# sevagh/xumx-sliCQ

Hardware: NVIDIA B200
Metric: sliCQT fwd+inv audio-sec/sec (higher is better)
Workload: dtype f32

## Files before the change

xumx_slicq_b200/csrc/slicq_api.cu:

```cuda
#include "slicq_common.cuh"
#include "../../include/slicq.h"

#include <math.h>
#include <stdio.h>
#include <stdlib.h>
#include <string.h>
#include <string>
#include <vector>
#include <algorithm>
#include <atomic>
#include <mutex>

#ifdef SLICQ_EMU
#include <condition_variable>
#include <mutex>
#include <thread>
thread_local dim3 threadIdx;
dim3 blockIdx, blockDim, gridDim;
static unsigned char slicq_emu_smem_buf[256 * 1024] __attribute__((aligned(16)));
unsigned char* slicq_emu_smem = slicq_emu_smem_buf;
namespace {
struct EmuBarrier {
    std::mutex m; std::condition_variable cv; int count = 0, gen = 0, n = 1;
    void wait() {
// ... 42 lines not shown
std::mutex g_prof_mutex;
#endif
struct ProfScope {
#ifndef SLICQ_EMU
    int kid; cudaStream_t s; cudaEvent_t a, b; bool on;
    ProfScope(int k, cudaStream_t st) : kid(k), s(st), on(g_prof) {
        if (on) { cudaEventCreate(&a); cudaEventCreate(&b); cudaEventRecord(a, s); }
    }
    ~ProfScope() {
        if (on) { cudaEventRecord(b, s); ProfRec r; r.kid = kid; r.a = a; r.b = b; std::lock_guard<std::mutex> lk(g_prof_mutex); g_prof_recs.push_back(r); }
    }
#else
    ProfScope(int, cudaStream_t) {}
#endif
};

int fail(int code, const std::string& msg) {
    g_err = msg;
    return code;
}

struct FftPlan { int M, kind, A, B, cost; };
const FftPlan kFftPlans[] = {
#define SLICQ_FFT_SIZE(M_, K_, A_, B_, C_) {M_, K_, A_, B_, C_},
#include "fft_sizes.inc"
#undef SLICQ_FFT_SIZE
};

const FftPlan* find_fft_plan(int M) {
    for (size_t i = 0; i < sizeof(kFftPlans) / sizeof(kFftPlans[0]); ++i)
        if (kFftPlans[i].M == M) return &kFftPlans[i];
    return nullptr;
}

int fft_smem_per_transform(const FftPlan& f) {
    if (f.kind == 1) return (f.M + 1) * 8;
    if (f.kind == 2) {
        const int bp = (f.B % 2 == 0) ? f.B + 1 : f.B;
        const int ap = (f.A % 2 == 0) ? f.A + 1 : f.A;
        const int a = f.A * bp, b = f.B * ap;
        return (a > b ? a : b) * 8;
    }
    return (f.M + f.A) * 8;
}

int fft_threads_per_transform(const FftPlan& f) {
    if (f.kind == 1) return 1;
    if (f.kind == 2) return f.B;
    return f.B * (f.A <= 41 ? 2 : (f.A <= 61 ? 3 : 4));
}

struct Bucket {
    int M, first_bin, n_bins, gt, tw_off, kind, A, B, smem_per_fft;
    int gap_first, gap_n;
    double cost;
};

template <class T> int upload(const std::vector<T>& h, const T** d, std::vector<void*>& owned) {
    void* p = nullptr;
    if (cudaMalloc(&p, h.size() * sizeof(T)) != cudaSuccess) return -1;
    if (cudaMemcpy(p, h.data(), h.size() * sizeof(T), cudaMemcpyHostToDevice) != cudaSuccess) return -1;
    owned.push_back(p);
    *d = reinterpret_cast<const T*>(p);
    return 0;
}

}

#define SLICQ_MAX_WAYS 8
struct slicq_plan {
    int L, N2, hop, J, sum_M;
    std::vector<int> bin_M, bin_pos, bin_coff;
    std::vector<Bucket> buckets;
    SlicqDeviceTables dev;
    std::vector<void*> owned;
    int bins_smem;
    int pad_l, pad_r;
    long long spec_stride_fwd;
    long long t_stride;
    long long chunk_bytes;
    int target_jobs;
    int min_iters;
    int only_bucket;
    long long split_units;
    int split_ways;
    mutable cudaStream_t side[SLICQ_MAX_WAYS];
    mutable cudaEvent_t ev_fork, ev_join[SLICQ_MAX_WAYS];
    mutable bool side_ready;
    mutable std::mutex split_mutex;
};

extern "C" int slicq_abi_version(void) { return SLICQ_ABI_VERSION; }
#ifdef SLICQ_EMU
extern "C" int slicq_build_kind(void) { return 1; }
#else
extern "C" int slicq_build_kind(void) { return 0; }
#endif
extern "C" const char* slicq_last_error(void) { return g_err.c_str(); }
extern "C" int64_t slicq_launch_count(void) { return g_launches.load(); }

extern "C" int slicq_profile_enable(int on) { g_prof = on != 0; return SLICQ_OK; }

extern "C" int slicq_profile_read(double* ms, int64_t* launches) {
    for (int i = 0; i < K_COUNT; ++i) { if (ms) ms[i] = 0.0; if (launches) launches[i] = 0; }
#ifndef SLICQ_EMU
    std::lock_guard<std::mutex> lk(g_prof_mutex);
    for (ProfRec& r : g_prof_recs) {
        float t = 0.f;
        if (cudaEventSynchronize(r.b) == cudaSuccess && cudaEventElapsedTime(&t, r.a, r.b) == cudaSuccess) {
            if (ms) ms[r.kid] += t;
            if (launches) launches[r.kid] += 1;
        }
        cudaEventDestroy(r.a); cudaEventDestroy(r.b);
    }
    g_prof_recs.clear();
#endif
    return SLICQ_OK;
}

extern "C" void slicq_plan_destroy(slicq_plan* p) {
    if (!p) return;
    if (p->side_ready) {
        for (int h = 0; h < SLICQ_MAX_WAYS; ++h) { cudaStreamDestroy(p->side[h]); cudaEventDestroy(p->ev_join[h]); }
        cudaEventDestroy(p->ev_fork);
    }
    for (void* q : p->owned) cudaFree(q);
    delete p;
}

extern "C" int slicq_plan_create(const slicq_tables* t, slicq_plan** out) {
    if (!t || !out) return fail(SLICQ_E_INVALID, "null argument");
    *out = nullptr;
    const int L = t->sl_len, J = t->n_bins;
    if (L <= 0 || L % 4 != 0) return fail(SLICQ_E_INVALID, "sl_len must be a positive multiple of 4");
    if (J < 2 || !t->bin_M || !t->bin_pos || !t->win_fwd || !t->win_inv || !t->tukey)
        return fail(SLICQ_E_INVALID, "missing tables");
    if (slicq_slice_smem_bytes(L) < 0) {
        char buf[160];
        snprintf(buf, sizeof buf, "slice length %d does not fit the slice kernels' shared memory (two buffers of sl_len/2 complex numbers)", L);
        return fail(SLICQ_E_UNSUPPORTED, buf);
    }
    slicq_plan* p = new slicq_plan();
    p->L = L; p->N2 = L / 2; p->hop = L / 2; p->J = J;
    p->bin_M.assign(t->bin_M, t->bin_M + J);
    p->bin_pos.assign(t->bin_pos, t->bin_pos + J);
    p->bin_coff.resize(J);
    int off = 0;
    for (int j = 0; j < J; ++j) {
        const int M = p->bin_M[j], pos = p->bin_pos[j];
        if (M < 4 || M % 4 != 0 || M > SLICQ_MAX_M || !find_fft_plan(M)) {
            delete p;
            return fail(SLICQ_E_UNSUPPORTED, "bin length M must be a multiple of 4 in [16, 292]");
        }
        if (pos % 2 != 0 || pos < 0 || pos > p->N2 || (j > 0 && pos <= p->bin_pos[j - 1])) {
            delete p;
            return fail(SLICQ_E_UNSUPPORTED, "bin positions must be even, increasing and within [0, L/2]");
        }
        p->bin_coff[j] = off;
        off += M;
    }
    p->sum_M = off;
    for (int j = 1; j < J - 1; ++j) {
        if (p->bin_pos[j] + p->bin_M[j] / 2 > p->N2) {
            delete p;
            return fail(SLICQ_E_UNSUPPORTED, "a bin below Nyquist reaches beyond it: the mirrored-bin pass above Nyquist is not implemented");
        }
    }
    int tw_off = 0;
    for (int j = 0; j < J; ++j) {
        if (!p->buckets.empty() && p->buckets.back().M == p->bin_M[j]) {
            p->buckets.back().n_bins++;
            continue;
        }
        const FftPlan* f = find_fft_plan(p->bin_M[j]);
        Bucket b;
        b.M = p->bin_M[j]; b.first_bin = j; b.n_bins = 1; b.tw_off = tw_off;
        b.kind = f->kind; b.A = f->A; b.B = f->B; b.smem_per_fft = fft_smem_per_transform(*f);
        b.gt = 1; b.cost = 0.0; b.gap_first = 0; b.gap_n = 0;
        tw_off += b.M;
        p->buckets.push_back(b);
    }
    if ((int)p->buckets.size() > SLICQ_MAX_BUCKETS) {
        delete p;
        return fail(SLICQ_E_UNSUPPORTED, "too many buckets");
    }
    p->bins_smem = 0;
    for (Bucket& b : p->buckets) {
        const FftPlan* f = find_fft_plan(b.M);
        const int nthr = slicq_bins_threads();
        int gt = nthr / (b.n_bins * fft_threads_per_transform(*f));
        if (gt < 1) gt = 1;
        static const int stage_kb = getenv("SLICQ_BINS_STAGE_KB") ? atoi(getenv("SLICQ_BINS_STAGE_KB")) : 48;
        while (gt > 1 && b.n_bins * gt * b.smem_per_fft > stage_kb * 1024) --gt;
        if (b.n_bins * fft_threads_per_transform(*f) > nthr) {
            delete p;
            return fail(SLICQ_E_UNSUPPORTED, "bucket has too many bins for one CTA");
        }
        b.gt = gt;
        const int sm = b.n_bins * gt * b.smem_per_fft + 4096 + (f->kind == 1 ? b.n_bins * b.M * 4 + b.n_bins * 12 + 32 : 0) + (f->kind == 3 ? b.n_bins * 12 + 16 : 0) +
                       (f->kind >= 2 ? b.M * 8 + b.n_bins * b.M * 4 + b.n_bins * 4 + 16 : 0);
        if (sm > p->bins_smem) p->bins_smem = sm;
        b.cost = (double)b.n_bins * f->cost;
    }

    std::vector<float> wf(p->sum_M), wi(p->sum_M), tuk(t->tukey, t->tukey + L);
    int pad_l = 0, pad_r = 0;
    for (int j = 0; j < J; ++j) {
        const int M = p->bin_M[j], o = p->bin_coff[j];
        const double sgn = ((p->bin_pos[j] / 2) % 2) ? -1.0 : 1.0;
        for (int mc = 0; mc < M; ++mc) {
            const int m = (mc + M / 2) % M;
            wf[o + mc] = (float)((double)t->win_fwd[o + m] * sgn / (double)M);
            wi[o + mc] = (float)((double)t->win_inv[o + m] * sgn * (double)M / (double)L);
        }
        pad_l = std::max(pad_l, M / 2 - p->bin_pos[j]);
        pad_r = std::max(pad_r, p->bin_pos[j] + M / 2 - 1 - p->N2);
    }
    pad_l = (pad_l + 1) & ~1;
    pad_r = (pad_r + 1) & ~1;
    if (pad_l > p->N2 / 2 || pad_r > p->N2 / 2) {
        delete p;
        return fail(SLICQ_E_UNSUPPORTED, "bins reach too far beyond DC / Nyquist");
    }
    p->pad_l = pad_l; p->pad_r = pad_r;
    int tw_lo = 0, tw_hi = L;
    while (tw_lo < L && tuk[tw_lo] == 0.f) ++tw_lo;
    while (tw_hi > tw_lo && tuk[tw_hi - 1] == 0.f) --tw_hi;
    std::vector<float2> post(p->N2 / 2 + 1), tw(tw_off);
    for (int k = 0; k <= p->N2 / 2; ++k) {
        const double a = -2.0 * M_PI * (double)k / (double)L;
        post[k] = make_float2((float)cos(a), (float)sin(a));
    }
    for (const Bucket& b : p->buckets)
        for (int j = 0; j < b.M; ++j) {
            const double a = -2.0 * M_PI * (double)j / (double)b.M;
            tw[b.tw_off + j] = make_float2((float)cos(a), (float)sin(a));
        }
    const int N2 = p->N2;
    const int pl_off = pad_l;
    const int pl_len = (pl_off + N2 + 2 + std::max(pad_r, 2) + 1) & ~1;
    std::vector<int> toff(J), ov(J, 0), ovoff(J, 0);
    int n_ovf = 0;
    for (int j = 0; j < J; ++j) {
        const int lo = p->bin_pos[j] - p->bin_M[j] / 2;
        toff[j] = (j & 1) * pl_len + pl_off + lo;
        if (j >= 2) {
            const int end_prev = p->bin_pos[j - 2] + p->bin_M[j - 2] / 2;
            ov[j] = std::max(0, end_prev - lo);
        }
        if (ov[j] > p->bin_M[j] || (ov[j] & 1)) { delete p; return fail(SLICQ_E_UNSUPPORTED, "unsupported overlap between bins of one plane"); }
        if (j >= 4 && p->bin_pos[j - 4] + p->bin_M[j - 4] / 2 > lo) { delete p; return fail(SLICQ_E_UNSUPPORTED, "more than 4 bins overlap at one spectrum position"); }
        ovoff[j] = 2 * pl_len + n_ovf;
        n_ovf += ov[j];
    }
    for (const Bucket& b : p->buckets)
        for (int j = b.first_bin; j < b.first_bin + b.n_bins; ++j)
            if ((b.kind == 2 && ov[j] > b.A) || (b.kind == 3 && ov[j] > b.B)) { delete p; return fail(SLICQ_E_UNSUPPORTED, "overlap between bins of one plane exceeds the first transform pass"); }
    p->t_stride = (2LL * pl_len + n_ovf + 1) & ~1LL;
    std::vector<int4> ex;
    {
        const bool fold = (t->flags & SLICQ_PLAN_ADJOINT_OF_ANALYSIS) != 0;
        std::vector<int> e0(N2 + 1, -1), e1(N2 + 1, -1), c0(N2 + 1, -1), c1(N2 + 1, -1);
        for (int j = 0; j < J; ++j)
            for (int m = 0; m < ov[j]; ++m) {
                int f = p->bin_pos[j] - p->bin_M[j] / 2 + m;
                const bool out = f < 0 || f > N2;
                if (out && !fold) continue;
                if (f < 0) f = -f;
                if (f > N2) f = 2 * N2 - f;
                std::vector<int>& a = out ? c0 : e0;
                std::vector<int>& b = out ? c1 : e1;
                if (a[f] < 0) a[f] = ovoff[j] + m;
                else if (b[f] < 0) b[f] = ovoff[j] + m;
                else { delete p; return fail(SLICQ_E_UNSUPPORTED, "more than two overflow entries at one spectrum position"); }
            }
        for (int f = 0; f <= N2; ++f)
            if (e0[f] >= 0) ex.push_back(int4{f, e0[f], e1[f], 0});
        for (int f = 0; f <= N2; ++f)
            if (c0[f] >= 0) ex.push_back(int4{f, c0[f], c1[f], 1});
        if (L == kTunedSliceLen && ex.size() > 0 && ex.back().w) {
            delete p;
            return fail(SLICQ_E_UNSUPPORTED, "adjoint of the analysis: overflow below DC / above Nyquist is not implemented in "
                                             "the tuned slice kernels (slice length 18060)");
        }
    }
    const int n_ex = (int)ex.size();
    if (ex.empty()) ex.push_back(int4{0, 0, -1, 0});
    std::vector<int2> gaps;
    {
        std::vector<std::vector<int2> > per_bucket(p->buckets.size());
        auto bucket_of = [&](int j) { for (size_t i = 0; i < p->buckets.size(); ++i) if (j >= p->buckets[i].first_bin && j < p->buckets[i].first_bin + p->buckets[i].n_bins) return (int)i; return 0; };
        for (int q = 0; q < 2; ++q) {
            std::vector<int> owner(pl_len, -1);
            int last = -1;
            for (int j = q; j < J; j += 2) {
                const int lo = std::max(0, pl_off + p->bin_pos[j] - p->bin_M[j] / 2), hi = std::min(pl_len, pl_off + p->bin_pos[j] + p->bin_M[j] / 2);
                for (int f = lo; f < hi; ++f) owner[f] = j;
                last = j;
            }
            if (last < 0) { delete p; return fail(SLICQ_E_UNSUPPORTED, "a bin plane is empty"); }
            for (int f = 0; f < pl_len;) {
                if (owner[f] >= 0) { ++f; continue; }
                int g = f;
                while (g < pl_len && owner[g] < 0) ++g;
                const int next = g < pl_len ? owner[g] : last;
                per_bucket[bucket_of(next)].push_back(int2{q * pl_len + f, g - f});
                f = g;
            }
        }
        for (size_t i = 0; i < p->buckets.size(); ++i) {
            p->buckets[i].gap_first = (int)gaps.size();
// ... 113 lines not shown
    const int64_t hh = p->L / 4;
    const int64_t nblk = (T + hh - 1) / hh;
    return (nblk + 1) / 2 + 1;
}

namespace {
long long bytes_per_unit(const slicq_plan* p, int inverse) {
    if (!inverse) return p->spec_stride_fwd * 8;
    return p->t_stride * 8;
}
long long chunk_units(const slicq_plan* p, int inverse) {
    long long c = p->chunk_bytes / bytes_per_unit(p, inverse);
    if (c >= 296) c -= c % 296;
    return c < 1 ? 1 : c;
}
}

namespace {
bool use_split(const slicq_plan* p, int64_t n_rows, int64_t n_slices) {
    return p->split_units > 0 && n_rows >= 2 && n_rows * n_slices >= p->split_units;
}
int split_ways(const slicq_plan* p, int64_t n_rows) { return (int)(n_rows < p->split_ways ? n_rows : p->split_ways); }
int64_t part_row0(int64_t n_rows, int ways, int h) { return n_rows * h / ways; }
size_t half_scratch(const slicq_plan* p, int64_t rows, int64_t n_slices, int inverse) {
    long long units = rows * n_slices;
    const long long c = chunk_units(p, inverse);
    if (units > c) units = c;
    return ((size_t)(units * bytes_per_unit(p, inverse)) + 511) & ~(size_t)255;
}
int ensure_side_streams(const slicq_plan* p) {
    if (p->side_ready) return 0;
    if (cudaEventCreateWithFlags(&p->ev_fork, cudaEventDisableTiming)) return -1;
    for (int h = 0; h < SLICQ_MAX_WAYS; ++h)
        if (cudaStreamCreateWithFlags(&p->side[h], cudaStreamNonBlocking) || cudaEventCreateWithFlags(&p->ev_join[h], cudaEventDisableTiming))
            return -1;
    p->side_ready = true;
    return 0;
}
}

extern "C" size_t slicq_scratch_bytes(const slicq_plan* p, int64_t n_rows, int64_t n_slices, int inverse) {
    if (!p || n_rows <= 0 || n_slices <= 0) return 0;
    if (use_split(p, n_rows, n_slices)) {
        const int ways = split_ways(p, n_rows);
        size_t total = 256;
        for (int h = 0; h < ways; ++h)
            total += half_scratch(p, part_row0(n_rows, ways, h + 1) - part_row0(n_rows, ways, h), n_slices, inverse);
        return total;
    }
    return half_scratch(p, n_rows, n_slices, inverse) + 256;
}

namespace {
int fill_bins_params(const slicq_plan* p, const slicq_bucket_view* views, SlicqBinsParams& bp, int n_rs,
                     const slicq_bucket_view* masks = nullptr, const slicq_bucket_view* norms = nullptr) {
    int jobs = 0;
    bp.n_buckets = (int)p->buckets.size();
    double total = 0.0;
    for (const Bucket& b : p->buckets) total += b.cost;
    const int target = p->target_jobs > 0 ? p->target_jobs : std::min(4440, std::max(1184, 4 * n_rs));
    for (size_t i = 0; i < p->buckets.size(); ++i) {
        const Bucket& b = p->buckets[i];
        SlicqBucketArg& a = bp.b[i];
        a.ptr = reinterpret_cast<float2*>(views[i].ptr);
        a.s_row = views[i].s_row; a.s_bin = views[i].s_bin; a.s_slice = views[i].s_slice;
        a.M = b.M; a.first_bin = b.first_bin; a.n_bins = b.n_bins; a.gt = b.gt; a.tw_off = b.tw_off;
        a.gap_first = b.gap_first; a.gap_n = b.gap_n;
        a.mptr = masks ? reinterpret_cast<const float*>(masks[i].ptr) : nullptr;
        a.nptr = norms ? reinterpret_cast<float*>(norms[i].ptr) : nullptr;
        const slicq_bucket_view* aux = masks ? masks : norms;
        a.ms_row = aux ? aux[i].s_row : 0; a.ms_bin = aux ? aux[i].s_bin : 0; a.ms_slice = aux ? aux[i].s_slice : 0;
        if (p->only_bucket >= 0 && (int)i != p->only_bucket) {
            a.units_per_job = b.gt; a.n_jobs = 0; a.job_start = jobs;
            continue;
        }
        const int groups = (n_rs + b.gt - 1) / b.gt;
        int nj = (int)(target * b.cost / total + 0.5);
        if (nj > groups / p->min_iters) nj = groups / p->min_iters;
        if (nj < 1) nj = 1;
        const int gpj = (groups + nj - 1) / nj;
        a.units_per_job = gpj * b.gt;
        a.n_jobs = (n_rs + a.units_per_job - 1) / a.units_per_job;
        a.job_start = jobs;
        jobs += a.n_jobs;
    }
    return jobs;
}
}

namespace {
int forward_one(const slicq_plan* p, const float* x, int64_t n_rows, int64_t x_row_stride,
                int64_t n_samples, int64_t t0, int64_t k0, int64_t n_slices,
                const slicq_bucket_view* buckets, const slicq_bucket_view* norms, void* scratch, cudaStream_t s);
int inverse_one(const slicq_plan* p, const slicq_bucket_view* buckets, const slicq_bucket_view* masks, int64_t x_rows,
                int64_t n_rows, int64_t n_slices, int64_t k0, float* y, int64_t y_row_stride, int64_t length,
                int64_t t0, float* halo_out, void* scratch, cudaStream_t s);

template <class F>
int run_split(const slicq_plan* p, int64_t n_rows, int64_t n_slices, int inverse, void* scratch, cudaStream_t s, F fn) {
    std::lock_guard<std::mutex> lock(p->split_mutex);
    if (ensure_side_streams(p)) return fail(SLICQ_E_CUDA, "cannot create internal streams");
    const int ways = split_ways(p, n_rows);
    unsigned char* base = reinterpret_cast<unsigned char*>(scratch);
    cudaEventRecord(p->ev_fork, s);
    int rc = 0;
    for (int h = 0; h < ways && rc == 0; ++h) {
        const int64_t r0 = part_row0(n_rows, ways, h), rows = part_row0(n_rows, ways, h + 1) - r0;
        cudaStreamWaitEvent(p->side[h], p->ev_fork, 0);
        rc = fn(r0, rows, base, p->side[h]);
        base += half_scratch(p, rows, n_slices, inverse);
        cudaEventRecord(p->ev_join[h], p->side[h]);
        cudaStreamWaitEvent(s, p->ev_join[h], 0);
    }
    return rc;
}
}

namespace {
int forward_impl(const slicq_plan* p, const float* x, int64_t n_rows, int64_t x_row_stride,
                 int64_t n_samples, int64_t t0, int64_t k0, int64_t n_slices,
                 const slicq_bucket_view* buckets, const slicq_bucket_view* norms, void* scratch, size_t scratch_bytes,
                 void* stream) {
    if (!p || !x || !buckets) return fail(SLICQ_E_INVALID, "null argument");
    if (n_rows <= 0 || n_slices <= 0 || n_samples < 0) return fail(SLICQ_E_INVALID, "bad shape");
    if (n_rows * n_slices > 0x7fffffffLL) return fail(SLICQ_E_INVALID, "too many (row,slice) units");
    if (scratch_bytes < slicq_scratch_bytes(p, n_rows, n_slices, 0) || !scratch)
        return fail(SLICQ_E_SCRATCH, "scratch buffer too small (see slicq_scratch_bytes)");
    if (reinterpret_cast<uintptr_t>(scratch) & 15) return fail(SLICQ_E_SCRATCH, "scratch buffer must be 16-byte aligned");
    for (size_t i = 0; i < p->buckets.size(); ++i)
        if (!buckets[i].ptr || (norms && !norms[i].ptr)) return fail(SLICQ_E_INVALID, "null bucket pointer");
    cudaStream_t s0 = reinterpret_cast<cudaStream_t>(stream);
    if (use_split(p, n_rows, n_slices)) {
        return run_split(p, n_rows, n_slices, 0, scratch, s0, [&](int64_t r0, int64_t rows, void* scr, cudaStream_t st) {
            std::vector<slicq_bucket_view> v(buckets, buckets + p->buckets.size()), nv;
            for (auto& b : v) b.ptr = reinterpret_cast<float2*>(b.ptr) + r0 * b.s_row;
            if (norms) {
                nv.assign(norms, norms + p->buckets.size());
                for (auto& b : nv) b.ptr = reinterpret_cast<float*>(b.ptr) + r0 * b.s_row;
            }
            return forward_one(p, x + r0 * x_row_stride, rows, x_row_stride, n_samples, t0, k0, n_slices, v.data(),
                               norms ? nv.data() : nullptr, scr, st);
        });
    }
    return forward_one(p, x, n_rows, x_row_stride, n_samples, t0, k0, n_slices, buckets, norms, scratch, s0);
}
}

extern "C" int slicq_forward(const slicq_plan* p, const float* x, int64_t n_rows, int64_t x_row_stride,
                             int64_t n_samples, int64_t t0, int64_t k0, int64_t n_slices,
                             const slicq_bucket_view* buckets, void* scratch, size_t scratch_bytes, void* stream) {
    return forward_impl(p, x, n_rows, x_row_stride, n_samples, t0, k0, n_slices, buckets, nullptr, scratch, scratch_bytes, stream);
}

extern "C" int slicq_forward_norm(const slicq_plan* p, const float* x, int64_t n_rows, int64_t x_row_stride,
                                  int64_t n_samples, int64_t t0, int64_t k0, int64_t n_slices,
                                  const slicq_bucket_view* buckets, const slicq_bucket_view* norms, void* scratch,
                                  size_t scratch_bytes, void* stream) {
    if (!norms) return fail(SLICQ_E_INVALID, "norms missing");
    return forward_impl(p, x, n_rows, x_row_stride, n_samples, t0, k0, n_slices, buckets, norms, scratch, scratch_bytes, stream);
}

namespace {
int forward_one(const slicq_plan* p, const float* x, int64_t n_rows, int64_t x_row_stride,
                int64_t n_samples, int64_t t0, int64_t k0, int64_t n_slices,
                const slicq_bucket_view* buckets, const slicq_bucket_view* norms, void* scratch, cudaStream_t s) {
    const long long units = n_rows * n_slices, cu = chunk_units(p, 0);
    float2* H = reinterpret_cast<float2*>((reinterpret_cast<uintptr_t>(scratch) + 255) & ~(uintptr_t)255);
    SlicqSliceParams sp;
    memset(&sp, 0, sizeof sp);
    sp.t = p->dev; sp.x = const_cast<float*>(x); sp.x_row_stride = x_row_stride; sp.T = n_samples; sp.t0 = t0; sp.k0 = k0;
    sp.spec = H; sp.spec_stride = p->spec_stride_fwd; sp.S = (int)n_slices;
    SlicqBinsParams* bp = new SlicqBinsParams();
    bp->t = p->dev; bp->spec = H; bp->spec_stride = p->spec_stride_fwd; bp->S = (int)n_slices;
    bp->k0 = (int)k0;
    int rc = 0;
    for (long long u0 = 0; u0 < units && rc == 0; u0 += cu) {
        const int n = (int)((units - u0 < cu) ? (units - u0) : cu);
        sp.n_rs = n; sp.rs0 = (int)u0;
        { ProfScope ps(K_SLICE_FWD, s); rc = slicq_launch_slice_fwd(&sp, s); }
        ++g_launches;
        if (rc) break;
        bp->n_rs = n; bp->rs0 = (int)u0;
        const int jobs = fill_bins_params(p, buckets, *bp, n, nullptr, norms);
        { ProfScope ps(K_BINS_FWD, s); rc = slicq_launch_bins(bp, jobs, p->bins_smem, 0, s); }
        ++g_launches;
        if (rc) break;
        if ((p->dev.adjoint & 1) && p->dev.n_mir > 0) {
            rc = slicq_launch_mirror_adj(bp, s);
            ++g_launches;
        }
    }
    delete bp;
    if (rc) {
        char buf[128];
        snprintf(buf, sizeof buf, "kernel launch failed: %s", rc > 0 ? cudaGetErrorString((cudaError_t)rc) : "unsupported");
        return fail(SLICQ_E_CUDA, buf);
    }
    return SLICQ_OK;
}
}

namespace {
std::vector<slicq_bucket_view> packed_views(const slicq_plan* p, void* base_, int64_t n_rows, int64_t n_slices, size_t elem) {
    std::vector<slicq_bucket_view> v(p->buckets.size());
    unsigned char* base = reinterpret_cast<unsigned char*>(base_);
    for (size_t i = 0; i < p->buckets.size(); ++i) {
        const Bucket& b = p->buckets[i];
        v[i].ptr = base;
        v[i].s_slice = b.M;
        v[i].s_bin = (int64_t)n_slices * b.M;
        v[i].s_row = (int64_t)b.n_bins * n_slices * b.M;
        base += (size_t)n_rows * b.n_bins * n_slices * b.M * elem;
    }
    return v;
}
}

extern "C" int slicq_forward_packed(const slicq_plan* p, const float* x, int64_t n_rows, int64_t x_row_stride,
                                    int64_t n_samples, int64_t t0, int64_t k0, int64_t n_slices, void* coefs,
                                    void* scratch, size_t scratch_bytes, void* stream) {
    if (!p || !coefs) return fail(SLICQ_E_INVALID, "null argument");
    std::vector<slicq_bucket_view> v = packed_views(p, coefs, n_rows, n_slices, 8);
    return slicq_forward(p, x, n_rows, x_row_stride, n_samples, t0, k0, n_slices, v.data(), scratch, scratch_bytes, stream);
}

extern "C" int slicq_forward_packed_norm(const slicq_plan* p, const float* x, int64_t n_rows, int64_t x_row_stride,
                                         int64_t n_samples, int64_t t0, int64_t k0, int64_t n_slices, void* coefs,
                                         void* norms, void* scratch, size_t scratch_bytes, void* stream) {
    if (!p || !coefs || !norms) return fail(SLICQ_E_INVALID, "null argument");
    std::vector<slicq_bucket_view> v = packed_views(p, coefs, n_rows, n_slices, 8);
    std::vector<slicq_bucket_view> nv = packed_views(p, norms, n_rows, n_slices, 4);
    return slicq_forward_norm(p, x, n_rows, x_row_stride, n_samples, t0, k0, n_slices, v.data(), nv.data(), scratch,
                              scratch_bytes, stream);
}

namespace {
// ... 1 lines not shown
                 int64_t n_rows, int64_t n_slices, int64_t k0, float* y, int64_t y_row_stride, int64_t length,
                 int64_t t0, float* halo_out, void* scratch, size_t scratch_bytes, void* stream) {
    if (!p || (!y && length > 0) || !buckets) return fail(SLICQ_E_INVALID, "null argument");
    if (n_rows <= 0 || n_slices <= 0 || length < 0) return fail(SLICQ_E_INVALID, "bad shape");
    if (n_rows * n_slices > 0x7fffffffLL) return fail(SLICQ_E_INVALID, "too many (row,slice) units");
    if (scratch_bytes < slicq_scratch_bytes(p, n_rows, n_slices, 1) || !scratch)
        return fail(SLICQ_E_SCRATCH, "scratch buffer too small (see slicq_scratch_bytes)");
    if (reinterpret_cast<uintptr_t>(scratch) & 15) return fail(SLICQ_E_SCRATCH, "scratch buffer must be 16-byte aligned");
    for (size_t i = 0; i < p->buckets.size(); ++i)
        if (!buckets[i].ptr) return fail(SLICQ_E_INVALID, "null bucket pointer");
    cudaStream_t s0 = reinterpret_cast<cudaStream_t>(stream);
    bool split = use_split(p, n_rows, n_slices);
    if (split && masks) {
        const int ways = split_ways(p, n_rows);
        for (int h = 1; h < ways; ++h) split = split && (part_row0(n_rows, ways, h) % x_rows == 0);
    }
    if (split) {
        return run_split(p, n_rows, n_slices, 1, scratch, s0, [&](int64_t r0, int64_t rows, void* scr, cudaStream_t st) {
            std::vector<slicq_bucket_view> v(buckets, buckets + p->buckets.size()), mv;
            if (masks) {
                mv.assign(masks, masks + p->buckets.size());
                for (auto& b : mv) b.ptr = reinterpret_cast<float*>(b.ptr) + r0 * b.s_row;
            } else {
                for (auto& b : v) b.ptr = reinterpret_cast<float2*>(b.ptr) + r0 * b.s_row;
            }
            return inverse_one(p, v.data(), masks ? mv.data() : nullptr, x_rows, rows, n_slices, k0, y + r0 * y_row_stride,
                               y_row_stride, length, t0, halo_out ? halo_out + r0 * p->hop : nullptr, scr, st);
        });
    }
    return inverse_one(p, buckets, masks, x_rows, n_rows, n_slices, k0, y, y_row_stride, length, t0, halo_out, scratch, s0);
}

int inverse_one(const slicq_plan* p, const slicq_bucket_view* buckets, const slicq_bucket_view* masks, int64_t x_rows,
                int64_t n_rows, int64_t n_slices, int64_t k0, float* y, int64_t y_row_stride, int64_t length,
                int64_t t0, float* halo_out, void* scratch, cudaStream_t s) {
    const long long units = n_rows * n_slices, cu = chunk_units(p, 1);
    const long long nu = units < cu ? units : cu;
    unsigned char* base = reinterpret_cast<unsigned char*>((reinterpret_cast<uintptr_t>(scratch) + 255) & ~(uintptr_t)255);
    float2* T = reinterpret_cast<float2*>(base);
    (void)nu;
    SlicqBinsParams* bp = new SlicqBinsParams();
    bp->t = p->dev; bp->spec = T; bp->spec_stride = p->t_stride; bp->S = (int)n_slices;
    bp->x_rows = masks ? (int)x_rows : 0;
    bp->k0 = (int)k0;
    SlicqSliceParams sp;
    memset(&sp, 0, sizeof sp);
    sp.t = p->dev; sp.k0 = k0; sp.spec = T; sp.spec_stride = p->t_stride; sp.S = (int)n_slices;
    sp.x = y; sp.x_row_stride = y_row_stride; sp.T = length; sp.t0 = t0; sp.halo_out = halo_out;
    int rc = 0;
    for (long long u0 = 0; u0 < units && rc == 0;) {
        long long n = (units - u0 < cu) ? (units - u0) : cu;
        while (n > 1 && u0 + n < units && ((u0 + n) % n_slices) != 0 && (((u0 + n) % n_slices) & 1) == 0) --n;
        bp->n_rs = (int)n; bp->rs0 = (int)u0;
        const int jobs = fill_bins_params(p, buckets, *bp, (int)n, masks);
        { ProfScope ps(K_BINS_INV, s); rc = slicq_launch_bins(bp, jobs, p->bins_smem, 1, s); }
        ++g_launches;
        if (rc) break;
        if (p->dev.n_mir > 0) {
            rc = slicq_launch_mirror_fix(bp, s);
            ++g_launches;
            if (rc) break;
        }
        sp.n_rs = (int)n; sp.rs0 = (int)u0;
        {
            ProfScope ps(K_SLICE_INV, s);
            sp.parity = 0; rc = slicq_launch_slice_inv(&sp, s);
            if (!rc) { sp.parity = 1; rc = slicq_launch_slice_inv(&sp, s); }
        }
        g_launches += 2;
        u0 += n;
    }
    delete bp;
    if (rc) {
        char buf[128];
        snprintf(buf, sizeof buf, "kernel launch failed: %s", rc > 0 ? cudaGetErrorString((cudaError_t)rc) : "unsupported");
        return fail(SLICQ_E_CUDA, buf);
    }
    return SLICQ_OK;
}
}

extern "C" int slicq_inverse(const slicq_plan* p, const slicq_bucket_view* buckets, int64_t n_rows,
                             int64_t n_slices, int64_t k0, float* y, int64_t y_row_stride, int64_t length,
                             int64_t t0, float* halo_out, void* scratch, size_t scratch_bytes, void* stream) {
    return inverse_impl(p, buckets, nullptr, 0, n_rows, n_slices, k0, y, y_row_stride, length, t0, halo_out,
                        scratch, scratch_bytes, stream);
}

extern "C" int slicq_inverse_masked(const slicq_plan* p, const slicq_bucket_view* mix, const slicq_bucket_view* masks,
                                    int64_t n_targets, int64_t n_rows, int64_t n_slices, int64_t k0, float* y,
                                    int64_t y_row_stride, int64_t length, int64_t t0, float* halo_out, void* scratch,
                                    size_t scratch_bytes, void* stream) {
    if (!masks || n_targets <= 0) return fail(SLICQ_E_INVALID, "masks / n_targets missing");
    if (p) for (size_t i = 0; i < p->buckets.size(); ++i)
        if (!masks[i].ptr) return fail(SLICQ_E_INVALID, "null mask pointer");
    return inverse_impl(p, mix, masks, n_rows, n_targets * n_rows, n_slices, k0, y, y_row_stride, length, t0, halo_out,
                        scratch, scratch_bytes, stream);
}
```

xumx_slicq_b200/csrc/slicq_fft_tile.cuh:

```cuda
#pragma once
#include "slicq_common.cuh"
#include "dft_codelets.cuh"

#if defined(SLICQ_PHASE_TIMING) && !defined(SLICQ_EMU)
__device__ long long* g_bins_phase_buf = nullptr;
#define BINS_T(v) const long long v = clock64()
#define BINS_T0(v) long long v = 0
#define BINS_SET(v) v = clock64()
#define BINS_COUNT() do { if (threadIdx.x == 0) ++bins_iters_; } while (0)
#define BINS_ACC(i, a, b) do { if (threadIdx.x == 0) bins_acc_[i] += (b) - (a); } while (0)
#define BINS_DECL long long bins_acc_[6] = {0, 0, 0, 0, 0, 0}; long long bins_iters_ = 0
#define BINS_FLUSH(M_) do { if (threadIdx.x == 0 && g_bins_phase_buf) { long long* o = g_bins_phase_buf + (long long)blockIdx.x * 8; \
        for (int q_ = 0; q_ < 6; ++q_) o[q_] = bins_acc_[q_]; o[6] = (M_) | (bins_iters_ << 16); o[7] = 1; } } while (0)
#else
#define BINS_T(v) do {} while (0)
#define BINS_T0(v) do {} while (0)
#define BINS_SET(v) do {} while (0)
#define BINS_COUNT() do {} while (0)
#define BINS_ACC(i, a, b) do {} while (0)
#define BINS_DECL do {} while (0)
#define BINS_FLUSH(M_) do {} while (0)
#endif

#ifdef SLICQ_DEBUG_TWRAP
// ... 229 lines not shown
            }
            dft<A, true>(v);
            y1[0] = v[0];
#pragma unroll
            for (int k1 = 1; k1 < A; ++k1)
                y1[k1 * BP] = cneg_if(cmul_conj(v[k1], twp[k1 * B]), k1 & 1);
        }
        BINS_T(t1_);
        __syncthreads();
        BINS_T(t2_);
        for (int t = tid; t < ng * j.F * A; t += blockDim.x) {
            const int slot = t / A, k1 = t - slot * A;
            const float2* src = sm + slot * PER + k1 * BP;
            float2 v[B];
#pragma unroll
            for (int n = 0; n < B; ++n) v[n] = src[n];
            dft<B, true>(v);
            float2* o = b.ptr + so[slot] + k1;
#pragma unroll
            for (int k2 = 0; k2 < B; ++k2) o[A * k2] = cneg_if(v[k2], (A * k2) & 1);
            if (b.nptr != nullptr) {
                float* on = b.nptr + so[256 + slot] + k1;
#pragma unroll
                for (int k2 = 0; k2 < B; ++k2) on[A * k2] = cmag(v[k2]);
            }
        }
        BINS_T(t3_);
        __syncthreads();
        BINS_T(t4_);
        BINS_ACC(1, t0_, t1_); BINS_ACC(2, t1_, t2_); BINS_ACC(3, t2_, t3_); BINS_ACC(4, t3_, t4_); BINS_ACC(5, t0_, t4_);
    }
    BINS_FLUSH(M);
}

template <int M, int A, int B>
SLICQ_DEVFN void syn_two_pass(const SlicqBinsParams& p, const SlicqBucketArg& b, const JobCtx& j, float2* sm) {
    static_assert(A * B == M, "bad split");
    constexpr int BP = (B % 2 == 0) ? B + 1 : B;
    constexpr int PER = A * BP;
    const int tid = threadIdx.x;
    const int per1 = j.F * B;
    const int gs1 = tid / per1, r1 = tid - gs1 * per1;
    const int f1 = r1 / B, n2 = r1 - f1 * B;
    const bool act1 = gs1 < j.gt;
    const bool odd = n2 & 1;
    int4* sc = reinterpret_cast<int4*>(sm);
    sm += SLICQ_SLOT_BYTES / sizeof(float2);
    for (int t = tid; t < j.gt * j.F; t += blockDim.x) {
        const int gs = t / j.F, f = t - gs * j.F;
        sc[t] = make_int4(gs | (f << 16), __ldg(p.t.bin_toff + j.first_bin + f), __ldg(p.t.bin_ov + j.first_bin + f),
                          __ldg(p.t.bin_ovoff + j.first_bin + f));
    }
    float2* y1 = sm + (gs1 * j.F + f1) * PER + n2;
    float2* twsm = sm + j.gt * j.F * PER;
    float* wsm = reinterpret_cast<float*>(twsm + M);
    const int coff_first = __ldg(p.t.bin_coff + j.first_bin);
    {
        const float2* __restrict__ tw = p.t.tw + b.tw_off;
        for (int t = tid; t < M; t += blockDim.x) { const int k1 = t / B, c2 = t - k1 * B; twsm[t] = __ldg(tw + c2 * k1); }
        for (int t = tid; t < j.F * M; t += blockDim.x) wsm[t] = __ldg(p.t.wi + coff_first + t);
    }
    const float2* twp = twsm + n2;
    __syncthreads();
    BINS_DECL;
    constexpr bool PIPE = (A + B <= SLICQ_PIPE_MAX);
    float2 v[A];
    int rowk[2] = {0, 0};
    auto request = [&](int base) {
        const int g = base + gs1;
        if (act1 && g < j.u1) {
            const int rs = SLICQ_CUNIT(j.rs0 + g);
            const int row = rs / j.S, k = rs - row * j.S;
            const int rowx = j.x_rows ? row % j.x_rows : row;
            const float2* src = b.ptr + rowx * b.s_row + f1 * b.s_bin + k * b.s_slice + n2;
#pragma unroll
            for (int n1 = 0; n1 < A; ++n1) v[n1] = (SLICQ_DBG_BINS & 1) ? make_float2((float)n1, (float)k) : src[B * n1];
            rowk[0] = row; rowk[1] = k;
        }
    };
    if (PIPE) request(j.u0);
    for (int base = j.u0; base < j.u1; base += j.gt) {
        BINS_T(t0_);
        BINS_T0(tl_);
        const int g = base + gs1;
        if (!PIPE) request(base);
        if (act1 && g < j.u1) {
#pragma unroll
            for (int n1 = 0; n1 < A; ++n1) v[n1] = cneg_if(v[n1], odd != (((B * n1) & 1) != 0));
            if (b.mptr != nullptr) {
                const float* msrc = b.mptr + rowk[0] * b.ms_row + f1 * b.ms_bin + rowk[1] * b.ms_slice + n2;
#pragma unroll
                for (int n1 = 0; n1 < A; ++n1) v[n1] = cscale(v[n1], msrc[B * n1]);
            }
            BINS_SET(tl_);
            if (!(SLICQ_DBG_BINS & 2)) dft<A, false>(v);
            y1[0] = v[0];
#pragma unroll
            for (int k1 = 1; k1 < A; ++k1) y1[k1 * BP] = cmul(v[k1], twp[k1 * B]);
        }
        if (PIPE && base + j.gt < j.u1) request(base + j.gt);
        BINS_T(t1_);
        __syncthreads();
        BINS_T(t2_);
        const int ng = (j.u1 - base < j.gt) ? (j.u1 - base) : j.gt;
        for (int t = tid; t < ng * j.F * A; t += blockDim.x) {
            const int slot = t / A, k1 = t - slot * A;
            const int4 c = sc[slot];
            const float2* src = sm + slot * PER + k1 * BP;
            float2 v[B];
#pragma unroll
            for (int n = 0; n < B; ++n) v[n] = src[n];
            if (!(SLICQ_DBG_BINS & 4)) dft<B, false>(v);
            if ((SLICQ_DBG_BINS & 8) && p.n_rs >= 0) continue;
            float2* row = p.spec + SLICQ_TROW(base + (c.x & 0xffff)) * p.spec_stride;
            float2* o = row + c.y + k1;
            const float* wp = wsm + (c.x >> 16) * M + k1;
            if (SLICQ_DBG_BINS & 16) {
                float2* oc = p.spec + SLICQ_TROW(base) * p.spec_stride + t;
                const int nt = ng * j.F * A;
#pragma unroll
                for (int k2 = 0; k2 < B; ++k2) oc[k2 * nt] = make_float2(v[k2].x * wp[A * k2], v[k2].y * wp[A * k2]);
                continue;
            }
            {
                const float w = wp[0];
                float2* o0 = (k1 < c.z) ? row + c.w + k1 : o;
                *o0 = make_float2(v[0].x * w, v[0].y * w);
            }
#pragma unroll
            for (int k2 = 1; k2 < B; ++k2) {
                const float w = wp[A * k2];
                o[A * k2] = make_float2(v[k2].x * w, v[k2].y * w);
            }
        }
        BINS_T(t3_);
        __syncthreads();
        BINS_T(t4_);
        BINS_ACC(0, t0_, tl_); BINS_ACC(1, tl_, t1_); BINS_ACC(2, t1_, t2_); BINS_ACC(3, t2_, t3_); BINS_ACC(4, t3_, t4_); BINS_ACC(5, t0_, t4_);
        BINS_COUNT();
    }
    BINS_FLUSH(M);
}

template <int M> struct PrimeSrcSyn {
    const float2* p;
    SLICQ_DEVFN cpx ld(int n) const { return cpx_ld(p + n); }
};
struct PrimeSrcAna {
    const float2* p; const float* w; int R;
    SLICQ_DEVFN cpx ld(int n) const { return cmulr(cpx_ld(p + R * n), w[R * n]); }
};
struct PrimeDstSyn {
    float2* o; const float* w; int R; int ovd;
    SLICQ_DEVFN void st(int k, cpx v) const { cpx_st(o + R * k + (k == 0 ? ovd : 0), cmulr(v, w[R * k])); }
};
struct PrimeDstAna {
    float2* o; const float2* tw; int RP, R;
    SLICQ_DEVFN void st(int k, cpx v) const { cpx_st(o + RP * k, k == 0 ? v : cmulw(v, tw[R * k])); }
};
constexpr __host__ __device__ int prime_parts(int P) { return P <= 41 ? 2 : (P <= 61 ? 3 : 4); }

template <int M, int P, int R>
SLICQ_DEVFN void ana_prime(const SlicqBinsParams& p, const SlicqBucketArg& b, const JobCtx& j, float* smf) {
    static_assert(P * R == M && R % 2 == 0, "bad split");
    constexpr int NP = (P <= 41 ? 2 : (P <= 61 ? 3 : 4)), RP = R + 1, PER = P * RP;
    typedef Dftp<P, NP, true> D;
    const int tid = threadIdx.x;
    long long* so = reinterpret_cast<long long*>(smf);
    float2* sm = reinterpret_cast<float2*>(smf + SLICQ_SLOT_BYTES / sizeof(float));
    float2* twsm = sm + (size_t)j.gt * j.F * PER;
    float* wsm = reinterpret_cast<float*>(twsm + M);
    int* hoff = reinterpret_cast<int*>(wsm + j.F * M);
    {
        const float2* __restrict__ tw = p.t.tw + b.tw_off;
        const int coff_first = __ldg(p.t.bin_coff + j.first_bin);
        for (int t = tid; t < M; t += blockDim.x) {
            const int k1 = t / R, c2 = t - k1 * R;
            float2 w = __ldg(tw + c2 * k1);
            w.y = -w.y;
            if (k1 & 1) { w.x = -w.x; w.y = -w.y; }
            twsm[t] = w;
        }
        for (int t = tid; t < j.F * M; t += blockDim.x) wsm[t] = __ldg(p.t.wf + coff_first + t);
        for (int t = tid; t < j.F; t += blockDim.x) hoff[t] = p.t.pad_l + __ldg(p.t.bin_pos + j.first_bin + t) - M / 2;
    }
    __syncthreads();
    for (int base = j.u0; base < j.u1; base += j.gt) {
        const int ng = (j.u1 - base < j.gt) ? (j.u1 - base) : j.gt;
        fill_slot_off(so, b, j, base, ng);
        const int ncol = ng * j.F * R, colp = (ncol + 31) & ~31;
        for (int t = tid; t < NP * colp; t += blockDim.x) {
            const int part = t / colp, c = t - part * colp;
            if (c >= ncol) continue;
            const int s = c / R, c2 = c - s * R;
            const int gs = s / j.F, f = s - gs * j.F;
            PrimeSrcAna src;
            src.p = p.spec + (long long)(base + gs) * p.spec_stride + hoff[f] + c2;
            src.w = wsm + f * M + c2; src.R = R;
            cpx o[D::NOUT];
            D::run(part, src, o);
            PrimeDstAna dst; dst.o = sm + s * PER + c2; dst.tw = twsm + c2; dst.RP = RP; dst.R = R;
            D::store(part, dst, o);
        }
        __syncthreads();
        for (int t = tid; t < ng * j.F * P; t += blockDim.x) {
            const int s = t / P, k1 = t - s * P;
            const float2* src = sm + s * PER + k1 * RP;
            cpx v[R];
#pragma unroll
            for (int n = 0; n < R; ++n) v[n] = cpx_ld(src + (n + R / 2) % R);
            dft<R, true>(v);
            float2* o = b.ptr + so[s] + k1;
#pragma unroll
            for (int k2 = 0; k2 < R; ++k2) cpx_st(o + P * k2, v[k2]);
            if (b.nptr != nullptr) {
                float* on = b.nptr + so[256 + s] + k1;
#pragma unroll
                for (int k2 = 0; k2 < R; ++k2) on[P * k2] = cmag(cpx_to(v[k2]));
            }
        }
        __syncthreads();
    }
}

template <int M, int P, int R>
SLICQ_DEVFN void syn_prime(const SlicqBinsParams& p, const SlicqBucketArg& b, const JobCtx& j, float* smf) {
    static_assert(P * R == M && R % 2 == 0, "bad split");
    constexpr int NP = (P <= 41 ? 2 : (P <= 61 ? 3 : 4));
    typedef Dftp<P, NP, false> D;
    const int tid = threadIdx.x;
    long long* so = reinterpret_cast<long long*>(smf);
    float2* sm = reinterpret_cast<float2*>(smf + SLICQ_SLOT_BYTES / sizeof(float));
    constexpr int SP = M + SLICQ_K3_PAD * P;
    float2* twsm = sm + (size_t)j.gt * j.F * (M + P);
    float* wsm = reinterpret_cast<float*>(twsm + M);
    const int coff_first = __ldg(p.t.bin_coff + j.first_bin);
    const int FM = j.F * M;
    int* tob = reinterpret_cast<int*>(wsm + FM);
    {
        const float2* __restrict__ tw = p.t.tw + b.tw_off;
        for (int t = tid; t < M; t += blockDim.x) {
            const int k1 = t / P, c2 = t - k1 * P;
            float2 w = __ldg(tw + c2 * k1);
            if (c2 & 1) { w.x = -w.x; w.y = -w.y; }
            twsm[t] = w;
        }
        for (int t = tid; t < FM; t += blockDim.x) wsm[t] = __ldg(p.t.wi + coff_first + t);
        for (int t = tid; t < j.F; t += blockDim.x) {
            tob[3 * t] = __ldg(p.t.bin_toff + j.first_bin + t);
            tob[3 * t + 1] = __ldg(p.t.bin_ov + j.first_bin + t);
            tob[3 * t + 2] = __ldg(p.t.bin_ovoff + j.first_bin + t);
        }
    }
    for (int base = j.u0; base < j.u1; base += j.gt) {
        const int ng = (j.u1 - base < j.gt) ? (j.u1 - base) : j.gt;
        fill_slot_off(so, b, j, base, ng);
        __syncthreads();
        for (int t = tid; t < ng * j.F * P; t += blockDim.x) {
            const int s = t / P, c2 = t - s * P;
            const float2* src = b.ptr + so[s] + c2;
            cpx v[R];
#pragma unroll
            for (int n1 = 0; n1 < R; ++n1) v[n1] = (SLICQ_DBG_BINS & 1) ? cpx_make((float)n1, (float)c2) : cpx_ld(src + P * n1);
            if (b.mptr != nullptr) {
                const float* msrc = b.mptr + so[256 + s] + c2;
#pragma unroll
                for (int n1 = 0; n1 < R; ++n1) v[n1] = cmulr(v[n1], msrc[P * n1]);
            }
            if (!(SLICQ_DBG_BINS & 2)) dft<R, false>(v);
            float2* o = sm + s * SP + c2;
            const float2* twp = twsm + c2;
#pragma unroll
            for (int k1 = 0; k1 < R; ++k1) cpx_st(o + k1 * P, cmulw(v[(k1 + R / 2) % R], twp[k1 * P]));
        }
        __syncthreads();
        const int ncol = ng * j.F * R, colp = (ncol + 31) & ~31;
        for (int t = tid; t < NP * colp; t += blockDim.x) {
            const int part = t / colp, c = t - part * colp;
            if (c >= ncol) continue;
            const int s = c / R, k1 = c - s * R;
            const int gs = s / j.F, f = s - gs * j.F;
            PrimeSrcSyn<M> src; src.p = sm + s * SP + k1 * P;
            cpx o[D::NOUT];
            if (!(SLICQ_DBG_BINS & 4)) D::run(part, src, o);
            else { for (int q = 0; q < D::NOUT; ++q) o[q] = src.ld(q); }
            if ((SLICQ_DBG_BINS & 8) && p.n_rs >= 0) continue;
            PrimeDstSyn dst;
            dst.o = p.spec + SLICQ_TROW(base + gs) * p.spec_stride + tob[3 * f] + k1;
            dst.w = wsm + f * M + k1; dst.R = R;
            dst.ovd = (k1 < tob[3 * f + 1]) ? tob[3 * f + 2] - tob[3 * f] : 0;
            D::store(part, dst, o);
        }
        __syncthreads();
    }
}
```

Baseline: 155,900.

## Stage synthesis outputs in shared memory and write rows with bulk async copies

The inverse (synthesis) bin kernels now write each transformed, windowed bin into a contiguous shared-memory run instead of storing strided elements directly to global memory. One thread per slot then issues TMA-style bulk shared-to-global copies, split into a main run and an overlap run. This needs extra shared memory and a separate group count and smem size for synthesis, plus alignment checks on the T layout. The prime path processes slots in chunks with extra barriers so it can reuse the staging buffer. The goal is coalesced, asynchronous global writes, at the cost of more syncs and possibly lower occupancy.

```diff
diff --git a/xumx_slicq_b200/csrc/slicq_api.cu b/xumx_slicq_b200/csrc/slicq_api.cu
--- a/xumx_slicq_b200/csrc/slicq_api.cu
+++ b/xumx_slicq_b200/csrc/slicq_api.cu
@@ -118,6 +118,7 @@
 
 struct Bucket {
     int M, first_bin, n_bins, gt, tw_off, kind, A, B, smem_per_fft;
+    int gt_syn;
     int gap_first, gap_n;
     double cost;
 };
@@ -141,6 +142,7 @@
     SlicqDeviceTables dev;
     std::vector<void*> owned;
     int bins_smem;
+    int bins_smem_syn;
     int pad_l, pad_r;
     long long spec_stride_fwd;
     long long t_stride;
@@ -242,7 +244,7 @@
         Bucket b;
         b.M = p->bin_M[j]; b.first_bin = j; b.n_bins = 1; b.tw_off = tw_off;
         b.kind = f->kind; b.A = f->A; b.B = f->B; b.smem_per_fft = fft_smem_per_transform(*f);
-        b.gt = 1; b.cost = 0.0; b.gap_first = 0; b.gap_n = 0;
+        b.gt = 1; b.gt_syn = 1; b.cost = 0.0; b.gap_first = 0; b.gap_n = 0;
         tw_off += b.M;
         p->buckets.push_back(b);
     }
@@ -251,6 +253,7 @@
         return fail(SLICQ_E_UNSUPPORTED, "too many buckets");
     }
     p->bins_smem = 0;
+    p->bins_smem_syn = 0;
     for (Bucket& b : p->buckets) {
         const FftPlan* f = find_fft_plan(b.M);
         const int nthr = slicq_bins_threads();
@@ -263,9 +266,17 @@
             return fail(SLICQ_E_UNSUPPORTED, "bucket has too many bins for one CTA");
         }
         b.gt = gt;
-        const int sm = b.n_bins * gt * b.smem_per_fft + 4096 + (f->kind == 1 ? b.n_bins * b.M * 4 + b.n_bins * 12 + 32 : 0) + (f->kind == 3 ? b.n_bins * 12 + 16 : 0) +
-                       (f->kind >= 2 ? b.M * 8 + b.n_bins * b.M * 4 + b.n_bins * 4 + 16 : 0);
-        if (sm > p->bins_smem) p->bins_smem = sm;
+        int gt_syn = gt, stage_syn = b.n_bins * gt * b.smem_per_fft;
+        if (f->kind == 2) {
+            const int per = (b.A * ((b.B % 2 == 0) ? b.B + 1 : b.B) + b.M) * 8;
+            while (gt_syn > 1 && b.n_bins * gt_syn * per > stage_kb * 1024) --gt_syn;
+            stage_syn = b.n_bins * gt_syn * per + 8;
+        }
+        b.gt_syn = gt_syn;
+        const int tables = 4096 + (f->kind == 1 ? b.n_bins * b.M * 4 + b.n_bins * 12 + 32 : 0) + (f->kind == 3 ? b.n_bins * 12 + 16 : 0) +
+                           (f->kind >= 2 ? b.M * 8 + b.n_bins * b.M * 4 + b.n_bins * 4 + 16 : 0);
+        p->bins_smem = std::max(p->bins_smem, b.n_bins * gt * b.smem_per_fft + tables);
+        p->bins_smem_syn = std::max(p->bins_smem_syn, stage_syn + tables);
         b.cost = (double)b.n_bins * f->cost;
     }
 
@@ -323,6 +334,11 @@
         for (int j = b.first_bin; j < b.first_bin + b.n_bins; ++j)
             if ((b.kind == 2 && ov[j] > b.A) || (b.kind == 3 && ov[j] > b.B)) { delete p; return fail(SLICQ_E_UNSUPPORTED, "overlap between bins of one plane exceeds the first transform pass"); }
     p->t_stride = (2LL * pl_len + n_ovf + 1) & ~1LL;
+    for (int j = 0; j < J; ++j)
+        if (((toff[j] | ov[j] | ovoff[j] | p->bin_M[j]) & 1) || (p->t_stride & 1)) {
+            delete p;
+            return fail(SLICQ_E_UNSUPPORTED, "synthesis rows of T are not 16-byte aligned for every bin");
+        }
     std::vector<int4> ex;
     {
         const bool fold = (t->flags & SLICQ_PLAN_ADJOINT_OF_ANALYSIS) != 0;
@@ -542,7 +558,7 @@
 }
 
 namespace {
-int fill_bins_params(const slicq_plan* p, const slicq_bucket_view* views, SlicqBinsParams& bp, int n_rs,
+int fill_bins_params(const slicq_plan* p, const slicq_bucket_view* views, SlicqBinsParams& bp, int n_rs, bool synth,
                      const slicq_bucket_view* masks = nullptr, const slicq_bucket_view* norms = nullptr) {
     int jobs = 0;
     bp.n_buckets = (int)p->buckets.size();
@@ -551,25 +567,26 @@
     const int target = p->target_jobs > 0 ? p->target_jobs : std::min(4440, std::max(1184, 4 * n_rs));
     for (size_t i = 0; i < p->buckets.size(); ++i) {
         const Bucket& b = p->buckets[i];
+        const int gt = synth ? b.gt_syn : b.gt;
         SlicqBucketArg& a = bp.b[i];
         a.ptr = reinterpret_cast<float2*>(views[i].ptr);
         a.s_row = views[i].s_row; a.s_bin = views[i].s_bin; a.s_slice = views[i].s_slice;
-        a.M = b.M; a.first_bin = b.first_bin; a.n_bins = b.n_bins; a.gt = b.gt; a.tw_off = b.tw_off;
+        a.M = b.M; a.first_bin = b.first_bin; a.n_bins = b.n_bins; a.gt = gt; a.tw_off = b.tw_off;
         a.gap_first = b.gap_first; a.gap_n = b.gap_n;
         a.mptr = masks ? reinterpret_cast<const float*>(masks[i].ptr) : nullptr;
         a.nptr = norms ? reinterpret_cast<float*>(norms[i].ptr) : nullptr;
         const slicq_bucket_view* aux = masks ? masks : norms;
         a.ms_row = aux ? aux[i].s_row : 0; a.ms_bin = aux ? aux[i].s_bin : 0; a.ms_slice = aux ? aux[i].s_slice : 0;
         if (p->only_bucket >= 0 && (int)i != p->only_bucket) {
-            a.units_per_job = b.gt; a.n_jobs = 0; a.job_start = jobs;
+            a.units_per_job = gt; a.n_jobs = 0; a.job_start = jobs;
             continue;
         }
-        const int groups = (n_rs + b.gt - 1) / b.gt;
+        const int groups = (n_rs + gt - 1) / gt;
         int nj = (int)(target * b.cost / total + 0.5);
         if (nj > groups / p->min_iters) nj = groups / p->min_iters;
         if (nj < 1) nj = 1;
         const int gpj = (groups + nj - 1) / nj;
-        a.units_per_job = gpj * b.gt;
+        a.units_per_job = gpj * gt;
         a.n_jobs = (n_rs + a.units_per_job - 1) / a.units_per_job;
         a.job_start = jobs;
         jobs += a.n_jobs;
@@ -671,7 +688,7 @@
         ++g_launches;
         if (rc) break;
         bp->n_rs = n; bp->rs0 = (int)u0;
-        const int jobs = fill_bins_params(p, buckets, *bp, n, nullptr, norms);
+        const int jobs = fill_bins_params(p, buckets, *bp, n, false, nullptr, norms);
         { ProfScope ps(K_BINS_FWD, s); rc = slicq_launch_bins(bp, jobs, p->bins_smem, 0, s); }
         ++g_launches;
         if (rc) break;
@@ -779,8 +796,8 @@
         long long n = (units - u0 < cu) ? (units - u0) : cu;
         while (n > 1 && u0 + n < units && ((u0 + n) % n_slices) != 0 && (((u0 + n) % n_slices) & 1) == 0) --n;
         bp->n_rs = (int)n; bp->rs0 = (int)u0;
-        const int jobs = fill_bins_params(p, buckets, *bp, (int)n, masks);
-        { ProfScope ps(K_BINS_INV, s); rc = slicq_launch_bins(bp, jobs, p->bins_smem, 1, s); }
+        const int jobs = fill_bins_params(p, buckets, *bp, (int)n, true, masks);
+        { ProfScope ps(K_BINS_INV, s); rc = slicq_launch_bins(bp, jobs, p->bins_smem_syn, 1, s); }
         ++g_launches;
         if (rc) break;
         if (p->dev.n_mir > 0) {
diff --git a/xumx_slicq_b200/csrc/slicq_fft_tile.cuh b/xumx_slicq_b200/csrc/slicq_fft_tile.cuh
--- a/xumx_slicq_b200/csrc/slicq_fft_tile.cuh
+++ b/xumx_slicq_b200/csrc/slicq_fft_tile.cuh
@@ -305,7 +305,8 @@
                           __ldg(p.t.bin_ovoff + j.first_bin + f));
     }
     float2* y1 = sm + (gs1 * j.F + f1) * PER + n2;
-    float2* twsm = sm + j.gt * j.F * PER;
+    float2* out = sm + ((j.gt * j.F * PER + 1) & ~1);
+    float2* twsm = out + j.gt * j.F * M;
     float* wsm = reinterpret_cast<float*>(twsm + M);
     const int coff_first = __ldg(p.t.bin_coff + j.first_bin);
     {
@@ -353,45 +354,41 @@
         }
         if (PIPE && base + j.gt < j.u1) request(base + j.gt);
         BINS_T(t1_);
+        if (tid < j.gt * j.F) bulk_wait_read();
         __syncthreads();
         BINS_T(t2_);
         const int ng = (j.u1 - base < j.gt) ? (j.u1 - base) : j.gt;
-        for (int t = tid; t < ng * j.F * A; t += blockDim.x) {
+        const int nslot = ng * j.F;
+        for (int t = tid; t < nslot * A; t += blockDim.x) {
             const int slot = t / A, k1 = t - slot * A;
-            const int4 c = sc[slot];
             const float2* src = sm + slot * PER + k1 * BP;
             float2 v[B];
 #pragma unroll
             for (int n = 0; n < B; ++n) v[n] = src[n];
             if (!(SLICQ_DBG_BINS & 4)) dft<B, false>(v);
-            if ((SLICQ_DBG_BINS & 8) && p.n_rs >= 0) continue;
-            float2* row = p.spec + SLICQ_TROW(base + (c.x & 0xffff)) * p.spec_stride;
-            float2* o = row + c.y + k1;
-            const float* wp = wsm + (c.x >> 16) * M + k1;
-            if (SLICQ_DBG_BINS & 16) {
-                float2* oc = p.spec + SLICQ_TROW(base) * p.spec_stride + t;
-                const int nt = ng * j.F * A;
-#pragma unroll
-                for (int k2 = 0; k2 < B; ++k2) oc[k2 * nt] = make_float2(v[k2].x * wp[A * k2], v[k2].y * wp[A * k2]);
-                continue;
-            }
-            {
-                const float w = wp[0];
-                float2* o0 = (k1 < c.z) ? row + c.w + k1 : o;
-                *o0 = make_float2(v[0].x * w, v[0].y * w);
-            }
-#pragma unroll
-            for (int k2 = 1; k2 < B; ++k2) {
+            const float* wp = wsm + (sc[slot].x >> 16) * M + k1;
+            float2* o = out + slot * M + k1;
+#pragma unroll
+            for (int k2 = 0; k2 < B; ++k2) {
                 const float w = wp[A * k2];
                 o[A * k2] = make_float2(v[k2].x * w, v[k2].y * w);
             }
         }
         BINS_T(t3_);
+        fence_proxy_async();
         __syncthreads();
         BINS_T(t4_);
+        if (tid < nslot && !((SLICQ_DBG_BINS & 8) && p.n_rs >= 0)) {
+            const int4 c = sc[tid];
+            float2* row = p.spec + SLICQ_TROW(base + (c.x & 0xffff)) * p.spec_stride;
+            const float2* run = out + tid * M;
+            bulk_s2g(row + c.y + c.z, run + c.z, (unsigned)(M - c.z) * 8u);
+            if (c.z > 0) bulk_s2g(row + c.w, run, (unsigned)c.z * 8u);
+        }
         BINS_ACC(0, t0_, tl_); BINS_ACC(1, tl_, t1_); BINS_ACC(2, t1_, t2_); BINS_ACC(3, t2_, t3_); BINS_ACC(4, t3_, t4_); BINS_ACC(5, t0_, t4_);
         BINS_COUNT();
     }
+    if (tid < j.gt * j.F) bulk_wait_read();
     BINS_FLUSH(M);
 }
 
@@ -404,8 +401,8 @@
     SLICQ_DEVFN cpx ld(int n) const { return cmulr(cpx_ld(p + R * n), w[R * n]); }
 };
 struct PrimeDstSyn {
-    float2* o; const float* w; int R; int ovd;
-    SLICQ_DEVFN void st(int k, cpx v) const { cpx_st(o + R * k + (k == 0 ? ovd : 0), cmulr(v, w[R * k])); }
+    float2* o; const float* w; int R;
+    SLICQ_DEVFN void st(int k, cpx v) const { cpx_st(o + R * k, cmulr(v, w[R * k])); }
 };
 struct PrimeDstAna {
     float2* o; const float2* tw; int RP, R;
@@ -505,9 +502,12 @@
             tob[3 * t + 2] = __ldg(p.t.bin_ovoff + j.first_bin + t);
         }
     }
+    static_assert(SP % 2 == 0, "output runs must start 16-byte aligned");
+    const int spr = ((int)(blockDim.x / NP) & ~31) / R;
     for (int base = j.u0; base < j.u1; base += j.gt) {
         const int ng = (j.u1 - base < j.gt) ? (j.u1 - base) : j.gt;
         fill_slot_off(so, b, j, base, ng);
+        if (tid < j.gt * j.F) bulk_wait_read();
         __syncthreads();
         for (int t = tid; t < ng * j.F * P; t += blockDim.x) {
             const int s = t / P, c2 = t - s * P;
@@ -527,23 +527,35 @@
             for (int k1 = 0; k1 < R; ++k1) cpx_st(o + k1 * P, cmulw(v[(k1 + R / 2) % R], twp[k1 * P]));
         }
         __syncthreads();
-        const int ncol = ng * j.F * R, colp = (ncol + 31) & ~31;
-        for (int t = tid; t < NP * colp; t += blockDim.x) {
-            const int part = t / colp, c = t - part * colp;
-            if (c >= ncol) continue;
-            const int s = c / R, k1 = c - s * R;
-            const int gs = s / j.F, f = s - gs * j.F;
-            PrimeSrcSyn<M> src; src.p = sm + s * SP + k1 * P;
+        const int nslot = ng * j.F;
+        for (int s0 = 0; s0 < nslot; s0 += spr) {
+            const int ncol = (nslot - s0 < spr ? nslot - s0 : spr) * R, colp = (ncol + 31) & ~31;
+            const int part = tid / colp, c = tid - part * colp;
+            const bool act = part < NP && c < ncol;
+            const int s = s0 + c / R, k1 = c - (c / R) * R;
             cpx o[D::NOUT];
-            if (!(SLICQ_DBG_BINS & 4)) D::run(part, src, o);
-            else { for (int q = 0; q < D::NOUT; ++q) o[q] = src.ld(q); }
-            if ((SLICQ_DBG_BINS & 8) && p.n_rs >= 0) continue;
-            PrimeDstSyn dst;
-            dst.o = p.spec + SLICQ_TROW(base + gs) * p.spec_stride + tob[3 * f] + k1;
-            dst.w = wsm + f * M + k1; dst.R = R;
-            dst.ovd = (k1 < tob[3 * f + 1]) ? tob[3 * f + 2] - tob[3 * f] : 0;
-            D::store(part, dst, o);
-        }
-        __syncthreads();
-    }
-}
+            if (act) {
+                PrimeSrcSyn<M> src; src.p = sm + s * SP + k1 * P;
+                if (!(SLICQ_DBG_BINS & 4)) D::run(part, src, o);
+                else { for (int q = 0; q < D::NOUT; ++q) o[q] = src.ld(q); }
+            }
+            __syncthreads();
+            if (act) {
+                PrimeDstSyn dst;
+                dst.o = sm + s * SP + k1; dst.w = wsm + (s % j.F) * M + k1; dst.R = R;
+                D::store(part, dst, o);
+            }
+        }
+        fence_proxy_async();
+        __syncthreads();
+        if (tid < nslot && !((SLICQ_DBG_BINS & 8) && p.n_rs >= 0)) {
+            const int gs = tid / j.F, f = tid - gs * j.F;
+            float2* row = p.spec + SLICQ_TROW(base + gs) * p.spec_stride;
+            const float2* run = sm + tid * SP;
+            const int ov = tob[3 * f + 1];
+            bulk_s2g(row + tob[3 * f] + ov, run + ov, (unsigned)(M - ov) * 8u);
+            if (ov > 0) bulk_s2g(row + tob[3 * f + 2], run, (unsigned)ov * 8u);
+        }
+    }
+    if (tid < j.gt * j.F) bulk_wait_read();
+}
```

Measured after the change: 146,600, median of 6. 0.94x the previous value.
